# lijx10/SO-Net

Measured on AMD Instinct MI355X. Metric: point-clouds/sec forward, ModelNet40 5k-pt 8x8 SOM, higher is better.
Workload: dtype f32 (operands split into fp16 pieces, 3 fp16 MFMAs per product, f32 accumulate; parity 1e-5)

## Files before the change

so-net_amd/csrc/pointresnet_fused.hip:

```cpp
#include "common.hpp"
#include <stdlib.h>
#include <type_traits>

namespace {


constexpr int PF_THREADS = 256, PF_WAVES = 4;
constexpr int WPTS = 64, TPTS = PF_WAVES * WPTS;
constexpr int T0 = 2, T1 = 4, T2 = 8, T3 = 12;
constexpr int KC2 = 2 * T0, KC3 = 2 * T1, KC4 = 2 * T0 + 2 * T2;
constexpr int MT4 = 3, NPASS = T3 / MT4;
constexpr int GS = 4;
constexpr int NSTG = 24;
constexpr int NTERM = 2;
constexpr int SL1 = 8 , SL2 = KC2 * GS * NTERM, SL3 = (T2 / GS) * KC3 * GS * NTERM;
constexpr int OFF1 = 0, OFF2 = SL1, OFF3 = SL1 + SL2, PRE = SL1 + SL2 + SL3;
constexpr int SL4 = KC4 * MT4 * NTERM;
constexpr int NSLICE = PRE + NPASS * SL4;
constexpr int NSTAGE = NSLICE / NSTG;
static_assert(PRE % NSTG == 0 && SL4 % NSTG == 0 && NSLICE % NSTG == 0, "layer 4 and every pass start on a stage boundary");
static_assert(NSTG % (NTERM * GS) == 0 && NSTG % (NTERM * MT4) == 0 && OFF2 % (NTERM * GS) == 0 && OFF3 % (NTERM * GS) == 0 && T1 == GS && T2 % GS == 0,
              "a step never straddles a stage boundary");
constexpr int NSW = NSTG / PF_WAVES;
static_assert(NSW == 6, "three DMA statements per wave and stage");
// ... 55 lines not shown
        constexpr int g = (I - 8) / 18, k = (I - 8) % 18;
        if constexpr (k < 4) { constexpr int e = 4 * g + k; v.x[e] = pin_fma(v.x[e], s.sc[e].x, s.sc[e].y); }
        else if constexpr (k < 6) { constexpr int e = 4 * g + 2 * (k - 4); if constexpr (RANGE) rm = pin_max3_i32(rm, v.x[e], v.x[e + 1]); }
        else if constexpr (k < 10) { constexpr int e = 4 * g + k - 6; v.x[e] = pin_relu_clamp32(v.x[e]); }
        else if constexpr (k < 12) { constexpr int P = 2 * g + (k - 10); v.h[P] = pin_cvt(v.x[2 * P], v.x[2 * P + 1]); }
        else if constexpr (k < 16) { constexpr int e = 4 * g + (k - 12); v.x[e] = (e & 1) ? pin_res_hi(v.h[e >> 1], v.x[e]) : pin_res_lo(v.h[e >> 1], v.x[e]); }
        else { constexpr int P = 2 * g + (k - 16); v.m[P] = pin_cvt(v.x[2 * P], v.x[2 * P + 1]); }
    } else {
        constexpr int w = I - 44;
        if constexpr (w < 4) agpr_write<R + w>(v.h[w]); else agpr_write<R + w>(v.m[w - 4]);
    }
}
template <int R, bool INPLACE, int I0, int I1, bool RANGE = true> __device__ __forceinline__ void job_ops(JobX &v, const JobSc &s, int &rm) {
    if constexpr (I0 < I1 && I0 < (INPLACE ? JOB_OPS_A : JOB_OPS_V)) { job_op<R, INPLACE, I0, RANGE>(v, s, rm); job_ops<R, INPLACE, I0 + 1, I1, RANGE>(v, s, rm); }
}
__device__ __forceinline__ JobOut job_result(const JobX &v) {
    JobOut o;
    o.h[0] = v.h[0]; o.h[1] = v.h[1]; o.h[2] = v.h[2]; o.h[3] = v.h[3];
    o.m[0] = v.m[0]; o.m[1] = v.m[1]; o.m[2] = v.m[2]; o.m[3] = v.m[3];
    return o;
}

template <int I0, int I1, class F> __device__ __forceinline__ void static_for(F &&f) {
    if constexpr (I0 < I1) { f(std::integral_constant<int, I0>{}); static_for<I0 + 1, I1>(f); }
}
#define SFOR(var, N) static_for<0, (N)>([&](auto var##_c_) __attribute__((always_inline)) { constexpr int var = decltype(var##_c_)::value;
#define SEND });

__global__ __launch_bounds__(256) void pointresnet_pack_kernel(const float *__restrict__ W1, const float *__restrict__ W2,
                                                                const float *__restrict__ W3, const float *__restrict__ W4,
                                                                int Cin0, uint4 *__restrict__ out, unsigned *__restrict__ trailer)
{
    const int t = blockIdx.x * 256 + threadIdx.x;
    if (t >= NSLICE * 64) return;
    RangeAcc wr = {0, 0u};
    const int lane = t & 63, s = t >> 6;
    const int i = lane & 31, h = lane >> 5;
    const float *W = nullptr;
    int Cin = 0, ct = 0, kc = 0, term = 0;
    bool chained = true, valid = true;
    if (s < OFF2) {
        const int u = s - OFF1; term = u % NTERM; kc = 0; ct = u / NTERM; W = W1; Cin = Cin0; chained = false; valid = u < T0 * NTERM;
    } else if (s < OFF3) {
        const int u = s - OFF2; term = u % NTERM; const int mt = (u / NTERM) % GS; kc = (u / (NTERM * GS)) % KC2;
        ct = (u / (NTERM * GS * KC2)) * GS + mt; W = W2; Cin = 32 * T0;
    } else if (s < PRE) {
        const int u = s - OFF3; term = u % NTERM; const int mt = (u / NTERM) % GS; kc = (u / (NTERM * GS)) % KC3;
        ct = (u / (NTERM * GS * KC3)) * GS + mt; W = W3; Cin = 32 * T1;
    } else {
        const int u = (s - PRE) % SL4, pass = (s - PRE) / SL4;
        term = u % NTERM; ct = pass * MT4 + (u / NTERM) % MT4; kc = u / (NTERM * MT4); W = W4; Cin = 32 * (T0 + T2);
    }
    unsigned w[4] = {0, 0, 0, 0};
    if (valid) {
#pragma unroll
        for (int p = 0; p < 4; ++p) {
            float v[2];
#pragma unroll
            for (int z = 0; z < 2; ++z) {
                const int e = 2 * p + z;
                const int c = chained ? kc * 16 + (e & 3) + 8 * (e >> 2) + 4 * h : kc * 16 + 8 * h + e;
                v[z] = c < Cin ? W[(long long)(ct * 32 + i) * Cin + c] : 0.f;
            }
            range_track(wr, 32.f * v[0], 32.f * v[1]);
            const float w0 = v[0] != v[0] ? v[0] : __builtin_fminf(__builtin_fmaxf(32.f * v[0], -F16_MAX32), F16_MAX32);
            const float w1 = v[1] != v[1] ? v[1] : __builtin_fminf(__builtin_fmaxf(32.f * v[1], -F16_MAX32), F16_MAX32);
            unsigned hh, ll;
            p16_split2(w0, w1, hh, ll);
            w[p] = term == 0 ? hh : ll;
        }
    }
    out[(long long)s * 64 + lane] = make_uint4(w[0], w[1], w[2], w[3]);
    range_publish(trailer, wave_umax(range_amax_bits(wr)), lane);
}

constexpr int NSLOT = 3;


struct AF { f16x8 h[GS], l[GS]; };

constexpr int SEG_SLOTS = 16;
constexpr int PCH = 32 * MT4;
constexpr unsigned SEG_INIT = 0x3B85FFFFu;

#ifdef SONET_PROF
constexpr int PROF_N = 32;
__device__ long long g_prof[1024 * PROF_N];
#define PROF_DECL long long prof_[PROF_N] = {}; const long long prof_rt0_ = (long long)__builtin_amdgcn_s_memrealtime(); long long prof_t_ = __builtin_readcyclecounter();
#define PROF_MARK(i) { const long long n_ = __builtin_readcyclecounter(); prof_[i] += n_ - prof_t_; prof_t_ = n_; }
#define PROF_T0 long long pt_ = __builtin_readcyclecounter();
#define PROF_T1(i) { const long long n_ = __builtin_readcyclecounter(); prof_[i] += n_ - pt_; pt_ = n_; }
#define PROF_DUMP prof_[31] = (long long)__builtin_amdgcn_s_memrealtime() - prof_rt0_;  if (lane == 0) { for (int i_ = 0; i_ < PROF_N; ++i_) g_prof[(blockIdx.x * PF_WAVES + wave) * PROF_N + i_] = prof_[i_]; }
#else
#define PROF_DECL
#define PROF_MARK(i)
#define PROF_T0
#define PROF_T1(i)
#define PROF_DUMP
#endif

#define PF_SB __builtin_amdgcn_sched_barrier(0);
#define PF_LDA(base, slice) __builtin_bit_cast(f16x8, (base)[(slice) * 64])
#define AG13(t, c) ((((t) * 2) + (c)) * 16)
#define AG2(t, c) (128 + (((t) * 2) + (c)) * 16)
#define PF_A8(n) "a" #n "0", "a" #n "1", "a" #n "2", "a" #n "3", "a" #n "4", "a" #n "5", "a" #n "6", "a" #n "7", "a" #n "8", "a" #n "9"
#define PF_CLAIM_AGPRS asm volatile("" ::: "a0", "a1", "a2", "a3", "a4", "a5", "a6", "a7", "a8", "a9", PF_A8(1), PF_A8(2), PF_A8(3), PF_A8(4), PF_A8(5), \
        PF_A8(6), PF_A8(7), PF_A8(8), PF_A8(9), PF_A8(10), PF_A8(11), PF_A8(12), PF_A8(13), PF_A8(14), PF_A8(15), PF_A8(16), PF_A8(17), PF_A8(18), PF_A8(19), \
        PF_A8(20), PF_A8(21), PF_A8(22), PF_A8(23), PF_A8(24), "a250", "a251", "a252", "a253", "a254", "a255");

template <bool SEGMAX, bool P16OUT = false>
__global__ __launch_bounds__(PF_THREADS, 1) void pointresnet_fused_kernel(
    const float *__restrict__ x, int Cin0, const uint4 *__restrict__ Wst, const float2 *__restrict__ affine_g ,
    float *__restrict__ y, int L, int tpc , long long ntiles,
    const int32_t *__restrict__ ids_sorted, const int32_t *__restrict__ pos0, unsigned *__restrict__ pooled, float *__restrict__ v0, int M,
    unsigned *__restrict__ partial ,
    unsigned *__restrict__ rlog ,
    void *__restrict__ yp = nullptr )
{
    static_assert(!(SEGMAX && P16OUT), "the pooled variant has no per-point output");
    RangeAcc yr4 = {0, 0u};
    __shared__ uint4 wsm[NSLOT * NSTG][64];
    __shared__ u32x4_t park[PF_WAVES][KC2][2][2][64];
    __shared__ uint4 w1s[T0 * NTERM][64];
    __shared__ __attribute__((aligned(16))) float2 aff[CH_TOTAL];
    __shared__ unsigned bins[SEGMAX ? SEG_SLOTS : 1][SEGMAX ? PCH : 1];

    PF_CLAIM_AGPRS
    const int lane = threadIdx.x & 63;
    const int wave = __builtin_amdgcn_readfirstlane(threadIdx.x >> 6);
    const int j = lane & 31, h = lane >> 5;
    bool l4_unit_lane = true;
    for (int c = threadIdx.x; c < CH_TOTAL; c += PF_THREADS) {
        const float2 v = affine_g[c];
        aff[c] = c < LB4 ? make_float2(v.x * ACC_TO_X32, 32.f * v.y) : make_float2(v.x * ACC_UNSCALE, v.y);
        if (c >= LB4 && v.x != 1.0f) l4_unit_lane = false;
    }
    if constexpr (SEGMAX) {
        for (int i = threadIdx.x; i < SEG_SLOTS * PCH; i += PF_THREADS) (&bins[0][0])[i] = SEG_INIT;
    }
    static_assert(T0 * NTERM * 64 == PF_THREADS, "one 16-byte piece of layer 1's slices per thread");
    w1s[threadIdx.x >> 6][threadIdx.x & 63] = Wst[OFF1 * 64 + threadIdx.x];
    const bool l4_unit = __syncthreads_and(l4_unit_lane) != 0;
    PROF_DECL

    unsigned vow = (unsigned)lane * 16u;
    const unsigned rowB = (unsigned)L * 4u;

    const unsigned wsm_lds = (unsigned)reinterpret_cast<size_t>(&wsm[0][0]);
    const char *dma_g = nullptr;
    unsigned dma_dst = 0;
    auto dma_setup = [&](int n, int slot) __attribute__((always_inline)) {
        const int sn = n % NSTAGE;
        dma_g = reinterpret_cast<const char *>(Wst) + (size_t)(sn * NSTG + wave * NSW) * 1024u;
        dma_dst = wsm_lds + (unsigned)(slot * NSTG + wave * NSW) * 1024u;
    };
    auto dma_pair = [&](auto tc) __attribute__((always_inline)) {
        constexpr int t = decltype(tc)::value;
        const char *g = dma_g + (t / 4) * 4096;
        const unsigned d = dma_dst + (unsigned)(t / 4) * 4096u;
        const unsigned vv = vow;
        if constexpr ((t % 4) == 0) asm volatile("s_mov_b32 m0, %2\n\ts_nop 4\n\tglobal_load_lds_dwordx4 %0, %1\n\tglobal_load_lds_dwordx4 %0, %1 offset:1024" :: "v"(vv), "s"(g), "s"(d) : "memory");
        else                        asm volatile("s_mov_b32 m0, %2\n\ts_nop 4\n\tglobal_load_lds_dwordx4 %0, %1 offset:2048\n\tglobal_load_lds_dwordx4 %0, %1 offset:3072" :: "v"(vv), "s"(g), "s"(d) : "memory");
    };
    auto stage_dma = [&](int n, int slot) __attribute__((always_inline)) {
        dma_setup(n, slot);
        dma_pair(std::integral_constant<int, 0>{}); dma_pair(std::integral_constant<int, 2>{}); dma_pair(std::integral_constant<int, 4>{});
// ... 17 lines not shown
        }
    };
    auto boundary = [&](auto flushc) __attribute__((always_inline)) {
        constexpr bool flush = decltype(flushc)::value;
        PROF_T0
        asm volatile("s_waitcnt vmcnt(0)" ::: "memory");
        PROF_T1(28)
        if constexpr (SEGMAX && flush) asm volatile("s_waitcnt lgkmcnt(0)" ::: "memory");
        __builtin_amdgcn_s_barrier();
        asm volatile("" ::: "memory");
        PROF_T1(29)
        if (!first_boundary) {
            n_cur += 1;
            const int t = slot_cur; slot_cur = slot_nxt; slot_nxt = slot_fill; slot_fill = t;
        }
        first_boundary = false;
        lds_cur = &wsm[slot_cur * NSTG][lane];
        lds_nxt = &wsm[slot_nxt * NSTG][lane];
        if constexpr (SEGMAX && flush) flush_bins();
        dma_setup(n_cur + 2, slot_fill);
    };

    AF af;
#define PF_STEP_HEAD(SIDX, SIDXN, FLUSH)                                                                 \
        constexpr int so_ = (SIDX) % NSTG, son_ = (SIDXN) % NSTG;                                        \
        if constexpr (so_ == 0) boundary(std::integral_constant<bool, (FLUSH)>{});                       \
        const uint4 *nb_ = son_ == 0 ? lds_nxt : lds_cur;
#define PF_STEP_A(NT, SIDX, NTN, SIDXN, AGB, BH0, BM0, BH1, BM1, ZERO, SLOT)                             \
    {                                                                                                    \
        PF_STEP_HEAD(SIDX, SIDXN, false)                                                                 \
        const f16x8 bh_[2] = {as_f16x8(BH0), as_f16x8(BH1)}, bm_[2] = {as_f16x8(BM0), as_f16x8(BM1)};    \
        PF_SB                                                                                            \
        SFOR(q, 2 * (NT)) constexpr int c = q / (NT), u = q % (NT);                                      \
            mfma_agpr<AGB(u, c), (ZERO)>(af.l[u], bh_[c]);                                               \
            if constexpr (so_ == 0 && q < 3) dma_pair(std::integral_constant<int, 2 * q>{});             \
            SLOT(q)                                                                                      \
            PF_SB                                                                                        \
        SEND                                                                                             \
        SFOR(q, 2 * (NT)) constexpr int c = q / (NT), u = q % (NT);                                      \
            mfma_agpr<AGB(u, c), false>(af.h[u], bm_[c]);                                                \
            SLOT(2 * (NT) + q)                                                                           \
            PF_SB                                                                                        \
        SEND                                                                                             \
        SFOR(u, NTN) af.l[u] = PF_LDA(nb_, son_ + NTERM * u + 1); SEND                                   \
        PF_SB                                                                                            \
        SFOR(q, 2 * (NT)) constexpr int c = q / (NT), u = q % (NT);                                      \
            mfma_agpr<AGB(u, c), false>(af.h[u], bh_[c]);                                                \
            SLOT(4 * (NT) + q)                                                                           \
            PF_SB                                                                                        \
        SEND                                                                                             \
        SFOR(u, NTN) af.h[u] = PF_LDA(nb_, son_ + NTERM * u); SEND                                       \
        PF_SB                                                                                            \
    }
#define PF_STEP_V(SIDX, SIDXN, ACC, FROMA, HN0, HN1, BH0, BM0, BH1, BM1, ZERO, FLUSH, SLOT)              \
    {                                                                                                    \
        PF_STEP_HEAD(SIDX, SIDXN, FLUSH)                                                                 \
        const f16x8 bh_[2] = {as_f16x8(BH0), as_f16x8(BH1)}, bm_[2] = {as_f16x8(BM0), as_f16x8(BM1)};    \
        constexpr int hn_[2] = {(HN0), (HN1)};                                                           \
        PF_SB                                                                                            \
        SFOR(q, 2 * MT4) constexpr int c = q / MT4, u = q % MT4;                                         \
            if constexpr (FROMA) mfma_va<hn_[c], SEGMAX>(ACC(u, c), af.l[u]);                            \
            else mfma_vv<(ZERO), SEGMAX>(ACC(u, c), af.l[u], bh_[c]);                                    \
            if constexpr (so_ == 0 && q < 3) dma_pair(std::integral_constant<int, 2 * q>{});             \
            SLOT(q)                                                                                      \
            PF_SB                                                                                        \
        SEND                                                                                             \
        SFOR(q, 2 * MT4) constexpr int c = q / MT4, u = q % MT4;                                         \
            if constexpr (FROMA) mfma_va<hn_[c] + 4, SEGMAX>(ACC(u, c), af.h[u]);                        \
            else mfma_vv<false, SEGMAX>(ACC(u, c), af.h[u], bm_[c]);                                     \
            SLOT(2 * MT4 + q)                                                                            \
            PF_SB                                                                                        \
        SEND                                                                                             \
        SFOR(u, MT4) af.l[u] = PF_LDA(nb_, son_ + NTERM * u + 1); SEND                                   \
        PF_SB                                                                                            \
        SFOR(q, 2 * MT4) constexpr int c = q / MT4, u = q % MT4;                                         \
            if constexpr (FROMA) mfma_va<hn_[c], SEGMAX>(ACC(u, c), af.h[u]);                            \
            else mfma_vv<false, SEGMAX>(ACC(u, c), af.h[u], bh_[c]);                                     \
            SLOT(4 * MT4 + q)                                                                            \
            PF_SB                                                                                        \
        SEND                                                                                             \
        SFOR(u, MT4) af.h[u] = PF_LDA(nb_, son_ + NTERM * u); SEND                                       \
        PF_SB                                                                                            \
    }
#define PF_LOAD_SC(scv, LB, t, Q)                                                                        \
    {                                                                                                    \
        const float4 *ap_ = reinterpret_cast<const float4 *>(&aff[(LB) + 32 * (t) + 16 * (Q) + 4 * h]);  \
        const float4 c0_ = ap_[0], c1_ = ap_[1], c2_ = ap_[4], c3_ = ap_[5];                             \
        scv.sc[0] = make_float2(c0_.x, c0_.y); scv.sc[1] = make_float2(c0_.z, c0_.w);                    \
        scv.sc[2] = make_float2(c1_.x, c1_.y); scv.sc[3] = make_float2(c1_.z, c1_.w);                    \
        scv.sc[4] = make_float2(c2_.x, c2_.y); scv.sc[5] = make_float2(c2_.z, c2_.w);                    \
        scv.sc[6] = make_float2(c3_.x, c3_.y); scv.sc[7] = make_float2(c3_.z, c3_.w);                    \
    }
#ifdef SONET_ABL_NOJOB
#define PF_JOBS_ON false
#else
#define PF_JOBS_ON true
#endif
#define PF_SLOT2(q, OPS, JOPS, INPL, R0, R1)                                                             \
    {                                                                                                    \
        if constexpr (PF_JOBS_ON && (q) >= 2 && (OPS) * ((q) - 2) < 2 * (JOPS)) {                                      \
            constexpr int i0_ = (OPS) * ((q) - 2), i1_ = i0_ + (OPS);                                    \
            if constexpr (i0_ < (JOPS)) job_ops<(R0), (INPL), i0_, (i1_ < (JOPS) ? i1_ : (JOPS))>(jx0_, sc_, rmax_); \
            if constexpr (i1_ > (JOPS)) job_ops<(R1), (INPL), (i0_ > (JOPS) ? i0_ - (JOPS) : 0), i1_ - (JOPS)>(jx1_, sc_, rmax_); \
        }                                                                                                \
    }
#define PF_SLOT1(q, OPS, JOPS, INPL, R0)                                                                 \
    {                                                                                                    \
        if constexpr (PF_JOBS_ON && (q) >= 2 && (OPS) * ((q) - 2) < (JOPS)) {                            \
            constexpr int i0_ = (OPS) * ((q) - 2);                                                       \
            job_ops<(R0), (INPL), i0_, i0_ + (OPS)>(jx0_, sc_, rmax_);                                   \
        }                                                                                                \
    }
    PROF_MARK(0)
    float xin_n[2][8];
    int nid_n[2] = {-1, -1}, n0_n = 0, nlast_n = 0, pos0_n = 0;
    auto prefetch_tile = [&](long long t) __attribute__((always_inline)) {
        t = t < ntiles ? t : ntiles - 1;
        const long long bb = t / tpc;
        const int t0 = (int)(t - bb * tpc) * TPTS;
        const __amdgpu_buffer_rsrc_t rxx = raw_buffer(x + bb * (long long)Cin0 * L, (int)((unsigned)Cin0 * rowB));
#pragma unroll
        for (int c = 0; c < 2; ++c) {
            const int ll0 = t0 + wave * WPTS + 32 * c;
            const bool pvv = ll0 + j < L;
            const int lcc = pvv ? ll0 + j : (ll0 < L ? ll0 : 0);
#pragma unroll
            for (int e = 0; e < 8; ++e)
                xin_n[c][e] = __builtin_bit_cast(float, __builtin_amdgcn_raw_buffer_load_b32(rxx, (unsigned)(8 * h * L + lcc) * 4u, (unsigned)e * rowB, 0));
            if constexpr (SEGMAX) nid_n[c] = pvv ? ids_sorted[bb * (long long)L + ll0 + j] : -1;
        }
        if constexpr (SEGMAX) {
            const int32_t *idb = ids_sorted + bb * (long long)L;
            n0_n = idb[t0];
            nlast_n = idb[(t0 + TPTS - 1 < L ? t0 + TPTS - 1 : L - 1)];
            pos0_n = pos0[bb];
        }
    };
    prefetch_tile(blockIdx.x);
    int rmax_ = 0;
    unsigned xin_r = 0u;
    u32x4_t *const park_w = &park[wave][0][0][0][lane];
#define PF_PARK(kc, c, piece) park_w[(((kc) * 2 + (c)) * 2 + (piece)) * 64]

    SFOR(u, T0) af.l[u] = PF_LDA(lds_cur, NTERM * u + 1); af.h[u] = PF_LDA(lds_cur, NTERM * u); SEND

    for (long long tile = blockIdx.x; tile < ntiles; tile += gridDim.x) {
        const long long b = tile / tpc;
        const int t0w = (int)(tile - b * tpc) * TPTS + wave * WPTS;
        bool pv[2]; int lc[2];
#pragma unroll
        for (int c = 0; c < 2; ++c) {
            const int l0 = t0w + 32 * c;
            pv[c] = l0 + j < L;
            lc[c] = pv[c] ? l0 + j : (l0 < L ? l0 : 0);
        }
        int nid[2] = {-1, -1}, n0 = 0, nslots = 0, jpos0[2] = {-1, -1};
        if constexpr (SEGMAX) {
            nid[0] = nid_n[0]; nid[1] = nid_n[1];
            n0 = n0_n;
            nslots = nlast_n - n0_n + 1 < SEG_SLOTS ? nlast_n - n0_n + 1 : SEG_SLOTS;
#pragma unroll
            for (int c = 0; c < 2; ++c) {
                const int p0 = pos0_n - (t0w + 32 * c);
                jpos0[c] = (p0 >= 0 && p0 < 32) ? p0 : -1;
            }
        }
        u32x4_t xh[2], xm[2];
#pragma unroll
        for (int c = 0; c < 2; ++c) {
#pragma unroll
            for (int p = 0; p < 4; ++p) {
                unsigned a0, a1;
                asm volatile("v_and_b32 %0, 0x7fffffff, %1" : "=v"(a0) : "v"(xin_n[c][2 * p]));
                asm volatile("v_and_b32 %0, 0x7fffffff, %1" : "=v"(a1) : "v"(xin_n[c][2 * p + 1]));
                asm volatile("v_max3_u32 %0, %0, %1, %2" : "+v"(xin_r) : "v"(a0), "v"(a1));
            }
            split_input(xin_n[c], xh[c], xm[c]);
        }
        PROF_MARK(1)
#define NOSLOT(q)
        PF_STEP_A(T0, OFF1, GS, OFF2, AG13, xh[0], xm[0], xh[1], xm[1], true, NOSLOT)
        JobOut a1[T0][2][2];
        {
            asm volatile("s_nop 15" ::: );
            JobSc sc_; JobX jx0_, jx1_;
            PF_LOAD_SC(sc_, LB1, 0, 0)
            job_ops<AG13(0, 0), false, 0, JOB_OPS_V>(jx0_, sc_, rmax_);
            job_ops<AG13(0, 1), false, 0, JOB_OPS_V>(jx1_, sc_, rmax_);
            a1[0][0][0] = job_result(jx0_); a1[0][0][1] = job_result(jx1_);
        }
        PROF_MARK(6)
        SFOR(k, KC2)
            constexpr int tk = k >> 1, qk = k & 1;
            constexpr int kn = k + 1, tn = (kn >> 1) & 1, qn = kn & 1;
            constexpr int sidx = OFF2 + k * NTERM * GS;
            JobSc sc_; JobX jx0_, jx1_;
            if constexpr (k + 1 < KC2) PF_LOAD_SC(sc_, LB1, tn, qn)
#define SLOT_L2(q) { if constexpr (k + 1 < KC2) { PF_SLOT2(q, 4, JOB_OPS_V, false, AG13(tn, 0) + 8 * qn, AG13(tn, 1) + 8 * qn) \
                       if constexpr ((q) == 23) { a1[tn][qn][0] = job_result(jx0_); a1[tn][qn][1] = job_result(jx1_); } } }
            PF_STEP_A(GS, sidx, GS, sidx + NTERM * GS, AG2, a1[tk][qk][0].h, a1[tk][qk][0].m, a1[tk][qk][1].h, a1[tk][qk][1].m, (k == 0), SLOT_L2)
#undef SLOT_L2
        SEND
        JobOut a2[T1][2][2];
        {
            asm volatile("s_nop 15" ::: );
            JobSc sc_; JobX jx0_, jx1_;
            PF_LOAD_SC(sc_, LB2, 0, 0)
            job_ops<AG2(0, 0), false, 0, JOB_OPS_V>(jx0_, sc_, rmax_);
            job_ops<AG2(0, 1), false, 0, JOB_OPS_V>(jx1_, sc_, rmax_);
            a2[0][0][0] = job_result(jx0_); a2[0][0][1] = job_result(jx1_);
        }
        PROF_MARK(7)
#define AG3A(u, c) AG13(u, c)
#define AG3B(u, c) AG13(GS + (u), c)
        u32x4_t pbh[2], pbm[2];
        SFOR(k, KC3)
            constexpr int tk = k >> 1, qk = k & 1;
            if constexpr (k + 1 == KC3) {
                pbh[0] = PF_PARK(0, 0, 0); pbm[0] = PF_PARK(0, 0, 1);
                pbh[1] = PF_PARK(0, 1, 0); pbm[1] = PF_PARK(0, 1, 1);
            }
            constexpr int kn = k + 1, tn = (kn >> 1) & 3, qn = kn & 1;
            constexpr int sidx = OFF3 + k * NTERM * GS;
            JobSc sc_; JobX jx0_, jx1_;
            if constexpr (k + 1 < KC3) PF_LOAD_SC(sc_, LB2, tn, qn)
#define SLOT_L3A(q) { if constexpr (k + 1 < KC3) { PF_SLOT2(q, 4, JOB_OPS_V, false, AG2(tn, 0) + 8 * qn, AG2(tn, 1) + 8 * qn) \
                        if constexpr ((q) == 23) { a2[tn][qn][0] = job_result(jx0_); a2[tn][qn][1] = job_result(jx1_); } } }
            PF_STEP_A(GS, sidx, GS, sidx + NTERM * GS, AG3A, a2[tk][qk][0].h, a2[tk][qk][0].m, a2[tk][qk][1].h, a2[tk][qk][1].m, (k == 0), SLOT_L3A)
#undef SLOT_L3A
            if constexpr (k < KC2) {
                PF_PARK(k, 0, 0) = a2[tk][qk][0].h; PF_PARK(k, 0, 1) = a2[tk][qk][0].m;
                PF_PARK(k, 1, 0) = a2[tk][qk][1].h; PF_PARK(k, 1, 1) = a2[tk][qk][1].m;
            }
        SEND
        PROF_MARK(8)
        float xagain[2][8];
        SFOR(k, KC3)
            constexpr int tk = k >> 1, qk = k & 1;
            constexpr int sidx = OFF3 + (KC3 + k) * NTERM * GS;
            constexpr int ntn = k + 1 < KC3 ? GS : MT4;
            constexpr bool cur_park = k < KC2, nxt_park = k + 1 < KC2;
            JobSc sc_; JobX jx0_, jx1_;
            PF_LOAD_SC(sc_, LB3, tk, qk)
            const u32x4_t ch0 = cur_park ? pbh[0] : a2[tk][qk][0].h, cm0 = cur_park ? pbm[0] : a2[tk][qk][0].m;
            const u32x4_t ch1 = cur_park ? pbh[1] : a2[tk][qk][1].h, cm1 = cur_park ? pbm[1] : a2[tk][qk][1].m;
            if constexpr (nxt_park) {
                pbh[0] = PF_PARK(k + 1, 0, 0); pbm[0] = PF_PARK(k + 1, 0, 1);
                pbh[1] = PF_PARK(k + 1, 1, 0); pbm[1] = PF_PARK(k + 1, 1, 1);
            }
            if constexpr (k + 1 == KC3) {
                const __amdgpu_buffer_rsrc_t rxx = raw_buffer(x + b * (long long)Cin0 * L, (int)((unsigned)Cin0 * rowB));
#pragma unroll
                for (int c = 0; c < 2; ++c)
#pragma unroll
                    for (int e = 0; e < 8; ++e)
                        xagain[c][e] = __builtin_bit_cast(float, __builtin_amdgcn_raw_buffer_load_b32(rxx, (unsigned)(8 * h * L + lc[c]) * 4u, (unsigned)e * rowB, 0));
            }
#define SLOT_L3B(q) { PF_SLOT2(q, 5, JOB_OPS_A, true, AG13(tk, 0) + 8 * qk, AG13(tk, 1) + 8 * qk) }
            PF_STEP_A(GS, sidx, ntn, sidx + NTERM * GS, AG3B, ch0, cm0, ch1, cm1, (k == 0), SLOT_L3B)
#undef SLOT_L3B
        SEND
        PROF_MARK(9)
        {
            f32x16 r1[T0][2];
            f16x8 wh[T0], wl[T0];
            SFOR(u, T0) wl[u] = __builtin_bit_cast(f16x8, w1s[NTERM * u + 1][lane]); wh[u] = __builtin_bit_cast(f16x8, w1s[NTERM * u][lane]); SEND
            u32x4_t xh0, xm0, xh1, xm1;
            split_input(xagain[0], xh0, xm0);
            split_input(xagain[1], xh1, xm1);
            const f16x8 bh_[2] = {as_f16x8(xh0), as_f16x8(xh1)}, bm_[2] = {as_f16x8(xm0), as_f16x8(xm1)};
            PF_SB
            SFOR(q, 2 * T0) constexpr int c = q / T0, u = q % T0; mfma_vv<true, false>(r1[u][c], wl[u], bh_[c]); PF_SB SEND
            SFOR(q, 2 * T0) constexpr int c = q / T0, u = q % T0; mfma_vv<false, false>(r1[u][c], wh[u], bm_[c]); PF_SB SEND
            SFOR(q, 2 * T0) constexpr int c = q / T0, u = q % T0; mfma_vv<false, false>(r1[u][c], wh[u], bh_[c]); PF_SB SEND
            asm volatile("s_nop 15" ::: );
            int rdummy = 0;
            SFOR(kk, KC2)
                constexpr int tk = kk >> 1, qk = kk & 1;
                JobSc sc_;
                PF_LOAD_SC(sc_, LB1, tk, qk)
                SFOR(c, 2)
                    JobX jx_;
                    SFOR(i, 8) jx_.x[i] = r1[tk][c][8 * qk + i]; SEND
                    job_ops<0, false, 8, JOB_OPS_V, false>(jx_, sc_, rdummy);
                    const JobOut o = job_result(jx_);
                    PF_PARK(kk, c, 0) = o.h; PF_PARK(kk, c, 1) = o.m;
                    if constexpr (kk == 0) { pbh[c] = o.h; pbm[c] = o.m; }
                SEND
            SEND
        }
        PROF_MARK(2)
        const __amdgpu_buffer_rsrc_t ry = raw_buffer(y ? y + b * (long long)(32 * T3) * L : x, y ? (int)((unsigned)(32 * T3) * rowB) : 0);
        const __amdgpu_buffer_rsrc_t ryp = raw_buffer(P16OUT ? static_cast<char *>(yp) + b * (long long)(2 * T3) * 64 * L : nullptr, P16OUT ? (int)((unsigned)(2 * T3) * 64u * (unsigned)L) : 0);
#define ACC4(u, c) acc[u][c]
#define PF_L4_BODY(JOBS)                                                                                 \
            SFOR(kc, KC4)                                                                                \
                constexpr int sidx = PRE + kc * NTERM * MT4;                                             \
                constexpr int kn = (kc + 1) % KC4;                                                       \
                constexpr bool cur_park = kc < KC2, nxt_park = kn < KC2;                                 \
                constexpr int t3 = cur_park ? 0 : (kc - KC2) >> 1, q3 = cur_park ? 0 : (kc - KC2) & 1;   \
                constexpr int jt = T2 / 2 + kc / 4, jq = (kc >> 1) & 1, jc = kc & 1;                     \
                constexpr bool job = (JOBS) && kc < 16;                                                  \
                JobSc sc_; JobX jx0_;                                                                    \
                if constexpr (job) PF_LOAD_SC(sc_, LB3, (job ? jt : 0), jq)                              \
                const u32x4_t ch0 = pbh[0], cm0 = pbm[0], ch1 = pbh[1], cm1 = pbm[1];                    \
                if constexpr (nxt_park) {                         \
                    pbh[0] = PF_PARK(kn, 0, 0); pbm[0] = PF_PARK(kn, 0, 1);                              \
                    pbh[1] = PF_PARK(kn, 1, 0); pbm[1] = PF_PARK(kn, 1, 1);                              \
                }                                                                                        \
                PF_STEP_V(sidx, sidx + NTERM * MT4, ACC4, !cur_park, AG13(t3, 0) + 8 * q3, AG13(t3, 1) + 8 * q3, ch0, cm0, ch1, cm1, (kc == 0), (kc == 0), SLOT_L4) \
            SEND
#define SLOT_L4(q) { if constexpr (job) { PF_SLOT1(q, 4, JOB_OPS_A, true, AG13((job ? jt : 0), jc) + 8 * jq) } }
        auto epilogue = [&](f32x16 (&acc)[MT4][2], const int pass) __attribute__((always_inline)) {
#ifdef SONET_ABL_NOEPI
            if (M != 12345) return;
#endif
            asm volatile("s_nop 15" ::: );
            if constexpr (SEGMAX) {
                float bias4[MT4];
#pragma unroll
                for (int mt = 0; mt < MT4; ++mt) {
                    const float2 ss = aff[LB4 + (pass * MT4 + mt) * 32 + j];
                    bias4[mt] = ss.y;
                    if (!l4_unit) {
#pragma unroll
                        for (int c = 0; c < 2; ++c)
#pragma unroll
                            for (int r = 0; r < 16; ++r) acc[mt][c][r] = __fmaf_rn(acc[mt][c][r], ss.x, ss.y);
                    }
                }
#pragma unroll
                for (int c = 0; c < 2; ++c) {
                    if (jpos0[c] >= 0) {
#pragma unroll
                        for (int r = 0; r < 16; ++r)
                            if ((r & 3) + 8 * (r >> 2) + 4 * h == jpos0[c]) {
#pragma unroll
                                for (int mt = 0; mt < MT4; ++mt) v0[b * (32 * T3) + (pass * MT4 + mt) * 32 + j] = l4_unit ? __fmaf_rn(acc[mt][c][r], ACC_UNSCALE, bias4[mt]) : acc[mt][c][r];
                            }
                    }
                    auto publish = [&](int node, float (&mx)[MT4]) __attribute__((always_inline)) {
                        if (l4_unit) {
#pragma unroll
                            for (int mt = 0; mt < MT4; ++mt) mx[mt] = __fmaf_rn(mx[mt], ACC_UNSCALE, bias4[mt]);
                        }
                        const int slot = node - n0;
                        if (slot < SEG_SLOTS) {
#pragma unroll
                            for (int mt = 0; mt < MT4; ++mt) atomicMax(&bins[slot][32 * mt + j], ord_f32(__float_as_uint(mx[mt])));
                        } else {
                            unsigned *gdst = pooled + ((long long)b * M + node) * (32 * T3) + pass * PCH;
#pragma unroll
                            for (int mt = 0; mt < MT4; ++mt) atomicMax(gdst + 32 * mt + j, ord_f32(__float_as_uint(mx[mt])));
                        }
                    };
                    unsigned remaining = (unsigned)__ballot(pv[c]);
                    if (remaining == 0xFFFFFFFFu) {
                        const int node_a = __builtin_amdgcn_readlane(nid[c], 0), node_b = __builtin_amdgcn_readlane(nid[c], 31);
                        const int e = __builtin_popcount((unsigned)__ballot(nid[c] == node_a));
                        if (node_a != node_b && __builtin_amdgcn_readlane(nid[c], e & 31) == node_b) {
                            float ma[MT4], mb[MT4];
#pragma unroll
                            for (int mt = 0; mt < MT4; ++mt) ma[mt] = mb[mt] = -__builtin_inff();
#pragma unroll
                            for (int r = 0; r < 16; r += 2) {
                                const int prow = (r & 3) + 8 * (r >> 2) + 4 * h;
                                const bool in0 = prow < e, in1 = prow + 1 < e;
#pragma unroll
                                for (int mt = 0; mt < MT4; ++mt) {
                                    const float a0 = in0 ? acc[mt][c][r] : -__builtin_inff(), a1 = in1 ? acc[mt][c][r + 1] : -__builtin_inff();
                                    const float b0 = in0 ? -__builtin_inff() : acc[mt][c][r], b1 = in1 ? -__builtin_inff() : acc[mt][c][r + 1];
                                    asm("v_max3_f32 %0, %1, %2, %3" : "=v"(ma[mt]) : "v"(ma[mt]), "v"(a0), "v"(a1));
                                    asm("v_max3_f32 %0, %1, %2, %3" : "=v"(mb[mt]) : "v"(mb[mt]), "v"(b0), "v"(b1));
                                }
                            }
                            publish(node_a, ma);
                            publish(node_b, mb);
                            remaining = 0u;
                        }
                    }
                    while (remaining != 0u) {
                        const int s0 = __builtin_ctz(remaining);
                        const int node = __builtin_amdgcn_readlane(nid[c], s0);
                        const unsigned segmask = (unsigned)__ballot(pv[c] && nid[c] == node);
                        remaining &= ~segmask;
                        const int e0 = s0 + __builtin_popcount(segmask);
                        const bool whole = (s0 == 0 && e0 == 32);
                        float mx[MT4];
                        if (whole) {
#pragma unroll
                            for (int mt = 0; mt < MT4; ++mt) {
                                float m;
                                asm("v_max_f32 %0, %1, %2" : "=v"(m) : "v"(acc[mt][c][0]), "v"(acc[mt][c][1]));
#pragma unroll
                                for (int r = 2; r < 16; r += 2) asm("v_max3_f32 %0, %1, %2, %3" : "=v"(m) : "v"(m), "v"(acc[mt][c][r]), "v"(acc[mt][c][r + 1]));
                                mx[mt] = m;
                            }
                        } else {
#pragma unroll
                            for (int mt = 0; mt < MT4; ++mt) mx[mt] = -__builtin_inff();
                            const unsigned nrows = (unsigned)(e0 - s0);
#pragma unroll
                            for (int r = 0; r < 16; r += 2) {
                                const int prow = (r & 3) + 8 * (r >> 2) + 4 * h;
                                const bool in0 = (unsigned)(prow - s0) < nrows, in1 = (unsigned)(prow + 1 - s0) < nrows;
#pragma unroll
                                for (int mt = 0; mt < MT4; ++mt) {
                                    const float v0_ = in0 ? acc[mt][c][r] : -__builtin_inff(), v1_ = in1 ? acc[mt][c][r + 1] : -__builtin_inff();
                                    asm("v_max3_f32 %0, %1, %2, %3" : "=v"(mx[mt]) : "v"(mx[mt]), "v"(v0_), "v"(v1_));
                                }
                            }
                        }
                        publish(node, mx);
                    }
                }
                pend_n = nslots * PCH;
                pend = partial + ((tile * NPASS + pass) * SEG_SLOTS) * (long long)PCH;
            } else {
#pragma unroll
                for (int c = 0; c < 2; ++c) {
                    if (!pv[c]) continue;
#pragma unroll
                    for (int mt = 0; mt < MT4; ++mt) {
                        const int ct = pass * MT4 + mt;
                        const unsigned so_tile = (unsigned)(ct * 32) * rowB;
                        float vv[16];
#pragma unroll
                        for (int r = 0; r < 16; ++r) {
                            const int orow = (r & 3) + 8 * (r >> 2);
                            const float2 ss = aff[LB4 + ct * 32 + orow + 4 * h];
                            const float v = __fmaf_rn(acc[mt][c][r], ss.x, ss.y);
                            vv[r] = v;
                            __builtin_amdgcn_raw_buffer_store_b32(__builtin_bit_cast(int, v), ry, (unsigned)(4 * h * L + lc[c]) * 4u,
                                                                  so_tile + (unsigned)orow * rowB, 0);
                        }
                        if constexpr (P16OUT) {
#pragma unroll
                            for (int q = 0; q < 2; ++q) {
                                unsigned hh[4], mm[4];
#pragma unroll
                                for (int p = 0; p < 4; ++p) {
                                    const float x0 = vv[8 * q + 2 * p], x1 = vv[8 * q + 2 * p + 1];
                                    range_track(yr4, x0, x1);
                                    p16_split_pair(x0, x1, hh[p], mm[p]);
                                }
                                const unsigned so = (unsigned)((ct * 2 + q) * 2) * (unsigned)L * 32u;
                                const u32x4_t hv = {hh[0], hh[1], hh[2], hh[3]}, mv = {mm[0], mm[1], mm[2], mm[3]};
                                __builtin_amdgcn_raw_buffer_store_b128(hv, ryp, (unsigned)(h * L + lc[c]) * 16u, so, 0);
                                __builtin_amdgcn_raw_buffer_store_b128(mv, ryp, (unsigned)(h * L + lc[c]) * 16u, so + (unsigned)L * 32u, 0);
                            }
                        }
                    }
                }
            }
        };
        {
            f32x16 acc[MT4][2];
            PF_L4_BODY(true)
            prefetch_tile(tile + gridDim.x);
            PROF_MARK(10)
            epilogue(acc, 0);
            PROF_MARK(4)
        }
        for (int pass = 1; pass < NPASS; ++pass) {
            f32x16 acc[MT4][2];
            PF_L4_BODY(false)
            PROF_MARK(3)
            epilogue(acc, pass);
            PROF_MARK(4)
        }
#undef SLOT_L4
    }
    asm volatile("s_waitcnt vmcnt(0)" ::: "memory");
    if constexpr (SEGMAX) {
        __syncthreads();
        flush_bins();
    }
    if (rlog != nullptr) {
        range_publish(rlog, wave_umax(xin_r), lane);
        unsigned rb = wave_umax((unsigned)(rmax_ > 0 ? rmax_ : 0));
        rb = rb > (5u << 23) ? rb - (5u << 23) : 0u;
        if constexpr (P16OUT) {
            const unsigned ob = wave_umax(range_amax_bits(yr4));
            rb = rb > ob ? rb : ob;
        }
        range_publish(rlog + 2, rb, lane);
        if (blockIdx.x == 0 && threadIdx.x == 0) atomicMax(rlog + 1, reinterpret_cast<const unsigned *>(Wst + (long long)NSLICE * 64)[0]);
    }
    PROF_MARK(5)
    PROF_DUMP
}

__global__ __launch_bounds__(256) void pooled_init_kernel(unsigned *__restrict__ pooled, long long n) {
    const long long t = (long long)blockIdx.x * 256 + threadIdx.x;
    if (t < n) pooled[t] = SEG_INIT;
}

__global__ __launch_bounds__(256) void pooled_decode_kernel(const unsigned *__restrict__ pooled, const unsigned *__restrict__ partial,
                                                             const int32_t *__restrict__ ids_sorted, const int32_t *__restrict__ node_off,
                                                             const int32_t *__restrict__ count, const float *__restrict__ v0,
                                                             float *__restrict__ out, int M, int L, int tpc,
                                                             uint4 *__restrict__ out_p16, unsigned *__restrict__ rlog)
{
    constexpr int C = 32 * T3;
    __shared__ float tile[32][33];
    const long long b = blockIdx.z;
    const int m0 = blockIdx.y * 32, c0 = blockIdx.x * 32;
    const int lx = threadIdx.x & 31, ly = threadIdx.x >> 5;
    const int c = c0 + lx;
    const int pass = c / PCH, cl = c - pass * PCH;
#pragma unroll
    for (int i = 0; i < 4; ++i) {
        const int m = m0 + ly + 8 * i;
        if (m < M) {
            unsigned key = pooled[(b * M + m) * C + c];
            const int cnt = count[b * M + m];
            if (cnt > 0) {
                const int off = node_off[b * M + m];
                for (int tl = off / TPTS; tl <= (off + cnt - 1) / TPTS; ++tl) {
                    const int slot = m - ids_sorted[b * L + tl * TPTS];
                    if (slot < SEG_SLOTS) {
                        const unsigned k2 = partial[((((b * tpc + tl) * NPASS + pass) * SEG_SLOTS) + slot) * (long long)PCH + cl];
                        key = k2 > key ? k2 : key;
                    }
                }
            }
            float v;
            if (key > SEG_INIT) v = __uint_as_float((key & 0x80000000u) ? (key ^ 0x80000000u) : ~key);
            else v = v0[b * C + c];
            tile[ly + 8 * i][lx] = v;
        }
    }
    __syncthreads();
#pragma unroll
    for (int i = 0; i < 4; ++i) {
        const int cc = c0 + ly + 8 * i, m = m0 + lx;
        if (m < M) out[(b * C + cc) * M + m] = tile[lx][ly + 8 * i];
    }
    if (out_p16 != nullptr && threadIdx.x < 128) {
        const int node = threadIdx.x & 31, qq = (threadIdx.x >> 6) & 1, hh = (threadIdx.x >> 5) & 1;
        const int m = m0 + node;
        RangeAcc xr = {0, 0u};
        if (m < M) {
            const long long BM = ((long long)gridDim.z * M + 127) / 128 * 128, l = b * M + m;
            float v[8];
#pragma unroll
            for (int e = 0; e < 8; ++e) v[e] = tile[node][16 * qq + 4 * hh + (e & 3) + 8 * (e >> 2)];
            unsigned hv[4], mv[4];
#pragma unroll
            for (int q = 0; q < 4; ++q) {
                range_track(xr, v[2 * q], v[2 * q + 1]);
                p16_split_pair(v[2 * q], v[2 * q + 1], hv[q], mv[q]);
            }
            const int kc = c0 / 16 + qq;
// ... 2 lines not shown
        }
        if (rlog != nullptr) range_publish(rlog + 2, wave_umax(range_amax_bits(xr)), (int)(threadIdx.x & 63));
    }
}

long long persistent_grid(long long ntiles, int cus) {
    static const int free_cus = [] { int v = 0; sonet::knob_int("SONET_FUSED_FREE_CUS", &v); return v; }();
    if (ntiles <= cus) return ntiles;
    if (free_cus == 0) return cus;
    const long long rounds = (ntiles + cus - 1) / cus;
    long long grid = (ntiles + rounds - 1) / rounds;
    if (free_cus > 0 && grid > cus - free_cus) grid = cus - free_cus > 1 ? cus - free_cus : 1;
    return free_cus > 0 || free_cus == -1 ? grid : cus;
}

}

extern "C" size_t sonet_pointresnet_pack_size(void) { return (size_t)NSLICE * 1024 + 64; }

extern "C" int sonet_pointresnet_pack(const float *W1, const float *W2, const float *W3, const float *W4, int Cin0,
                                      void *stream_out, sonet_stream_t stream)
{
    const char *what = "sonet_pointresnet_pack";
    SONET_REQUIRE(W1 && W2 && W3 && W4 && stream_out, "%s: NULL pointer", what);
    SONET_REQUIRE(Cin0 >= 1 && Cin0 <= 16, "%s: Cin0=%d must be in [1, 16]", what, Cin0);
    unsigned *trailer = reinterpret_cast<unsigned *>(reinterpret_cast<char *>(stream_out) + (size_t)NSLICE * 1024);
    if (hipMemsetAsync(trailer, 0, 64, sonet::as_stream(stream)) != hipSuccess) return sonet::fail(SONET_ERR_LAUNCH, "%s: memset failed", what);
    hipLaunchKernelGGL(pointresnet_pack_kernel, dim3(sonet::ceil_div(NSLICE * 64, 256)), dim3(256), 0, sonet::as_stream(stream),
                       W1, W2, W3, W4, Cin0, reinterpret_cast<uint4 *>(stream_out), trailer);
    return sonet::launched(what);
}

extern "C" int sonet_pointresnet_fused_f32(const float *x, int Cin0, const void *wstream, const float *affine,
                                           float *y, int B, int L, sonet_stream_t stream)
{
    const char *what = "sonet_pointresnet_fused_f32";
    SONET_REQUIRE(x && wstream && affine && y, "%s: NULL pointer", what);
    SONET_REQUIRE(B > 0 && L > 0 && Cin0 >= 1 && Cin0 <= 16, "%s: bad size B=%d L=%d Cin0=%d", what, B, L, Cin0);
    if ((double)(32 * T3) * L * 4.0 >= 4.0e9) return sonet::fail(SONET_ERR_UNSUPPORTED, "%s: a per-cloud panel exceeds 4 GiB", what);
    const int tpc = sonet::ceil_div(L, TPTS);
    const long long ntiles = (long long)B * tpc;
    const long long grid = persistent_grid(ntiles, sonet::cu_count(1));
    hipLaunchKernelGGL((pointresnet_fused_kernel<false>), dim3((unsigned)grid), dim3(PF_THREADS), 0, sonet::as_stream(stream),
                       x, Cin0, reinterpret_cast<const uint4 *>(wstream), reinterpret_cast<const float2 *>(affine), y, L, tpc, ntiles,
                       (const int32_t *)nullptr, (const int32_t *)nullptr, (unsigned *)nullptr, (float *)nullptr, 0, (unsigned *)nullptr, sonet::range_log());
    return sonet::launched(what);
}

extern "C" int sonet_pointresnet_fused_p16_f32(const float *x, int Cin0, const void *wstream, const float *affine,
                                               float *y, void *yp, int B, int L, sonet_stream_t stream)
{
    const char *what = "sonet_pointresnet_fused_p16_f32";
    SONET_REQUIRE(x && wstream && affine && yp, "%s: NULL pointer", what);
    SONET_REQUIRE(B > 0 && L > 0 && Cin0 >= 1 && Cin0 <= 16, "%s: bad size B=%d L=%d Cin0=%d", what, B, L, Cin0);
    if ((double)(32 * T3) * L * 4.0 >= 2.0e9) return sonet::fail(SONET_ERR_UNSUPPORTED, "%s: a per-cloud panel exceeds 2 GiB", what);
    const int tpc = sonet::ceil_div(L, TPTS);
    const long long ntiles = (long long)B * tpc;
    const long long grid = persistent_grid(ntiles, sonet::cu_count(1));
    hipLaunchKernelGGL((pointresnet_fused_kernel<false, true>), dim3((unsigned)grid), dim3(PF_THREADS), 0, sonet::as_stream(stream),
                       x, Cin0, reinterpret_cast<const uint4 *>(wstream), reinterpret_cast<const float2 *>(affine), y, L, tpc, ntiles,
                       (const int32_t *)nullptr, (const int32_t *)nullptr, (unsigned *)nullptr, (float *)nullptr, 0, (unsigned *)nullptr, sonet::range_log(), yp);
    return sonet::launched(what);
}

extern "C" size_t sonet_pointresnet_pool_ws_size(int B, int L, int M)
{
    if (B <= 0 || L <= 0 || M <= 0) return 0;
    const long long ntiles = (long long)B * sonet::ceil_div(L, TPTS);
    return (size_t)((long long)B * M * (32 * T3) + ntiles * NPASS * SEG_SLOTS * PCH) * 4 + (size_t)B * (32 * T3) * 4;
}

static int fused_pool_impl(const char *what, const float *x_sorted, int Cin0, const void *wstream, const float *affine,
                           const int32_t *ids_sorted, const int32_t *pos0, const int32_t *node_off,
                           const int32_t *count, void *ws, float *out, void *out_p16, int B, int L, int M, sonet_stream_t stream)
{
    SONET_REQUIRE(x_sorted && wstream && affine && ids_sorted && pos0 && node_off && count && ws && out, "%s: NULL pointer", what);
    SONET_REQUIRE(B > 0 && L > 0 && M > 0 && Cin0 >= 1 && Cin0 <= 16, "%s: bad size B=%d L=%d M=%d Cin0=%d", what, B, L, M, Cin0);
    if (B > 65535) return sonet::fail(SONET_ERR_UNSUPPORTED, "%s: B=%d > 65535", what, B);
    if (16.0 * L * 4.0 >= 4.0e9) return sonet::fail(SONET_ERR_UNSUPPORTED, "%s: a per-cloud input panel of 16 rows exceeds 4 GiB", what);
    hipStream_t st = sonet::as_stream(stream);
    const long long npool = (long long)B * M * (32 * T3);
    const int tpc = sonet::ceil_div(L, TPTS);
    const long long ntiles = (long long)B * tpc;
    unsigned *pooled_ws = reinterpret_cast<unsigned *>(ws);
    unsigned *partial_ws = pooled_ws + npool;
    float *v0_ws = reinterpret_cast<float *>(partial_ws + ntiles * NPASS * SEG_SLOTS * PCH);
    hipLaunchKernelGGL(pooled_init_kernel, dim3((unsigned)sonet::ceil_div64(npool, 256)), dim3(256), 0, st, pooled_ws, npool);
    const long long grid = persistent_grid(ntiles, sonet::cu_count(1));
    hipLaunchKernelGGL((pointresnet_fused_kernel<true>), dim3((unsigned)grid), dim3(PF_THREADS), 0, st,
                       x_sorted, Cin0, reinterpret_cast<const uint4 *>(wstream), reinterpret_cast<const float2 *>(affine), (float *)nullptr,
                       L, tpc, ntiles, ids_sorted, pos0, pooled_ws, v0_ws, M, partial_ws, sonet::range_log());
    hipLaunchKernelGGL(pooled_decode_kernel, dim3((unsigned)(32 * T3 / 32), (unsigned)sonet::ceil_div(M, 32), (unsigned)B), dim3(256), 0, st,
                       pooled_ws, partial_ws, ids_sorted, node_off, count, v0_ws, out, M, L, tpc, reinterpret_cast<uint4 *>(out_p16), sonet::range_log());
    return sonet::launched(what);
}

extern "C" int sonet_pointresnet_fused_pool_f32(const float *x_sorted, int Cin0, const void *wstream, const float *affine,
                                                const int32_t *ids_sorted, const int32_t *pos0, const int32_t *node_off,
                                                const int32_t *count, void *ws, float *out, int B, int L, int M, sonet_stream_t stream)
{
    return fused_pool_impl("sonet_pointresnet_fused_pool_f32", x_sorted, Cin0, wstream, affine, ids_sorted, pos0, node_off, count, ws, out, nullptr, B, L, M, stream);
}

extern "C" int sonet_pointresnet_fused_pool_p16_f32(const float *x_sorted, int Cin0, const void *wstream, const float *affine,
                                                    const int32_t *ids_sorted, const int32_t *pos0, const int32_t *node_off,
                                                    const int32_t *count, void *ws, float *out, void *out_p16, int B, int L, int M, sonet_stream_t stream)
{
    const char *what = "sonet_pointresnet_fused_pool_p16_f32";
    SONET_REQUIRE(out_p16, "%s: NULL pointer", what);
    return fused_pool_impl(what, x_sorted, Cin0, wstream, affine, ids_sorted, pos0, node_off, count, ws, out, out_p16, B, L, M, stream);
}

#ifdef SONET_PROF
extern "C" int sonet_prof_read(long long *host, int n)
{
    return hipMemcpyFromSymbol(host, HIP_SYMBOL(g_prof), sizeof(long long) * (size_t)n, 0, hipMemcpyDeviceToHost) == hipSuccess ? 0 : 1;
}
#endif
```

Before: 78030.

## Overlap segment max-pool reduction with next pass MFMAs and track tile coordinates incrementally

Adds an optional path, on only when SONET_VARIANTS is defined, that interleaves the per-pass segment max-pool reduction (max3, scale and bias, ordered-int encode, LDS atomicMax) for wave-uniform tiles into the MFMA slots of the last and first layer-4 steps, in place of running a separate epilogue. Separately, the segmax kernel now keeps batch and tile indices incrementally instead of 64-bit divisions per tile, and the host rejects tile counts of 2^31 or more. The overlap path adds register pressure and inline asm. Without the define, only the incremental indexing takes effect.

Result: no change. 77930 (-0.1%).

```diff
diff --git a/so-net_amd/csrc/pointresnet_fused.hip b/so-net_amd/csrc/pointresnet_fused.hip
--- a/so-net_amd/csrc/pointresnet_fused.hip
+++ b/so-net_amd/csrc/pointresnet_fused.hip
@@ -161,6 +161,11 @@
 constexpr int SEG_SLOTS = 16;
 constexpr int PCH = 32 * MT4;
 constexpr unsigned SEG_INIT = 0x3B85FFFFu;
+#ifdef SONET_VARIANTS
+constexpr bool PF_POOL_OVERLAP = true;
+#else
+constexpr bool PF_POOL_OVERLAP = false;
+#endif
 
 #ifdef SONET_PROF
 constexpr int PROF_N = 32;
@@ -344,6 +349,30 @@
         SFOR(u, MT4) af.h[u] = PF_LDA(nb_, son_ + NTERM * u); SEND                                       \
         PF_SB                                                                                            \
     }
+#define PF_STEP_VC(SIDX, SIDXN, ACC, FROMA, HN0, HN1, BH0, BM0, BH1, BM1, ZERO, SLOT)                    \
+    {                                                                                                    \
+        PF_STEP_HEAD(SIDX, SIDXN, false)                                                                 \
+        const f16x8 bh_[2] = {as_f16x8(BH0), as_f16x8(BH1)}, bm_[2] = {as_f16x8(BM0), as_f16x8(BM1)};    \
+        constexpr int hn_[2] = {(HN0), (HN1)};                                                           \
+        PF_SB                                                                                            \
+        SFOR(q, 2 * MT4) constexpr int c = q / MT4, u = q % MT4;                                         \
+            if constexpr (FROMA) mfma_va<hn_[c], SEGMAX>(ACC(u, c), af.l[u]);                            \
+            else mfma_vv<(ZERO), SEGMAX>(ACC(u, c), af.l[u], bh_[c]);                                    \
+            if constexpr (so_ == 0 && q < 3) dma_pair(std::integral_constant<int, 2 * q>{});             \
+            SLOT(3 * q)                                                                                  \
+            PF_SB                                                                                        \
+            if constexpr (FROMA) mfma_va<hn_[c] + 4, SEGMAX>(ACC(u, c), af.h[u]);                        \
+            else mfma_vv<false, SEGMAX>(ACC(u, c), af.h[u], bm_[c]);                                     \
+            SLOT(3 * q + 1)                                                                              \
+            PF_SB                                                                                        \
+            if constexpr (c == 1) { af.l[u] = PF_LDA(nb_, son_ + NTERM * u + 1); PF_SB }                 \
+            if constexpr (FROMA) mfma_va<hn_[c], SEGMAX>(ACC(u, c), af.h[u]);                            \
+            else mfma_vv<false, SEGMAX>(ACC(u, c), af.h[u], bh_[c]);                                     \
+            SLOT(3 * q + 2)                                                                              \
+            PF_SB                                                                                        \
+            if constexpr (c == 1) { af.h[u] = PF_LDA(nb_, son_ + NTERM * u); PF_SB }                     \
+        SEND                                                                                             \
+    }
 #define PF_LOAD_SC(scv, LB, t, Q)                                                                        \
     {                                                                                                    \
         const float4 *ap_ = reinterpret_cast<const float4 *>(&aff[(LB) + 32 * (t) + 16 * (Q) + 4 * h]);  \
@@ -376,10 +405,24 @@
     PROF_MARK(0)
     float xin_n[2][8];
     int nid_n[2] = {-1, -1}, n0_n = 0, nlast_n = 0, pos0_n = 0;
+    int g_q = 0, g_r = 0, b_last = 0, b_n = 0, tl_n = 0;
+    if constexpr (SEGMAX) {
+        g_q = (int)(gridDim.x / (unsigned)tpc); g_r = (int)(gridDim.x % (unsigned)tpc);
+        b_last = (int)((unsigned)(ntiles - 1) / (unsigned)tpc);
+        b_n = (int)(blockIdx.x / (unsigned)tpc); tl_n = (int)(blockIdx.x % (unsigned)tpc);
+    }
     auto prefetch_tile = [&](long long t) __attribute__((always_inline)) {
-        t = t < ntiles ? t : ntiles - 1;
-        const long long bb = t / tpc;
-        const int t0 = (int)(t - bb * tpc) * TPTS;
+        long long bb;
+        int t0;
+        if constexpr (SEGMAX) {
+            if (t >= ntiles) { b_n = b_last; tl_n = tpc - 1; }
+            bb = b_n;
+            t0 = tl_n * TPTS;
+        } else {
+            t = t < ntiles ? t : ntiles - 1;
+            bb = t / tpc;
+            t0 = (int)(t - bb * tpc) * TPTS;
+        }
         const __amdgpu_buffer_rsrc_t rxx = raw_buffer(x + bb * (long long)Cin0 * L, (int)((unsigned)Cin0 * rowB));
 #pragma unroll
         for (int c = 0; c < 2; ++c) {
@@ -407,8 +450,8 @@
     SFOR(u, T0) af.l[u] = PF_LDA(lds_cur, NTERM * u + 1); af.h[u] = PF_LDA(lds_cur, NTERM * u); SEND
 
     for (long long tile = blockIdx.x; tile < ntiles; tile += gridDim.x) {
-        const long long b = tile / tpc;
-        const int t0w = (int)(tile - b * tpc) * TPTS + wave * WPTS;
+        const long long b = SEGMAX ? (long long)b_n : tile / tpc;
+        const int t0w = (SEGMAX ? tl_n : (int)(tile - b * tpc)) * TPTS + wave * WPTS;
         bool pv[2]; int lc[2];
 #pragma unroll
         for (int c = 0; c < 2; ++c) {
@@ -426,6 +469,17 @@
                 const int p0 = pos0_n - (t0w + 32 * c);
                 jpos0[c] = (p0 >= 0 && p0 < 32) ? p0 : -1;
             }
+        }
+        bool fastw = false;
+        int fslot[2] = {0, 0};
+        unsigned fmask = 0u;
+        if constexpr (SEGMAX && PF_POOL_OVERLAP) {
+            const int na0 = __builtin_amdgcn_readfirstlane(nid[0]), na1 = __builtin_amdgcn_readfirstlane(nid[1]);
+            const bool w0 = __ballot(pv[0] && nid[0] == na0) == ~0ull, w1 = __ballot(pv[1] && nid[1] == na1) == ~0ull;
+            const int n0u = __builtin_amdgcn_readfirstlane(n0);
+            fastw = __builtin_amdgcn_readfirstlane((int)(l4_unit && w0 && w1 && jpos0[0] < 0 && jpos0[1] < 0 && na1 - n0u < SEG_SLOTS)) != 0;
+            fslot[0] = fastw ? na0 - n0u : 0; fslot[1] = fastw ? na1 - n0u : 0;
+            fmask = fastw ? 0xFFFFFFFFu : 0u;
         }
         u32x4_t xh[2], xm[2];
 #pragma unroll
@@ -555,7 +609,7 @@
         const __amdgpu_buffer_rsrc_t ry = raw_buffer(y ? y + b * (long long)(32 * T3) * L : x, y ? (int)((unsigned)(32 * T3) * rowB) : 0);
         const __amdgpu_buffer_rsrc_t ryp = raw_buffer(P16OUT ? static_cast<char *>(yp) + b * (long long)(2 * T3) * 64 * L : nullptr, P16OUT ? (int)((unsigned)(2 * T3) * 64u * (unsigned)L) : 0);
 #define ACC4(u, c) acc[u][c]
-#define PF_L4_BODY(JOBS)                                                                                 \
+#define PF_L4_BODY(JOBS, OVL)                                                                            \
             SFOR(kc, KC4)                                                                                \
                 constexpr int sidx = PRE + kc * NTERM * MT4;                                             \
                 constexpr int kn = (kc + 1) % KC4;                                                       \
@@ -570,7 +624,17 @@
                     pbh[0] = PF_PARK(kn, 0, 0); pbm[0] = PF_PARK(kn, 0, 1);                              \
                     pbh[1] = PF_PARK(kn, 1, 0); pbm[1] = PF_PARK(kn, 1, 1);                              \
                 }                                                                                        \
-                PF_STEP_V(sidx, sidx + NTERM * MT4, ACC4, !cur_park, AG13(t3, 0) + 8 * q3, AG13(t3, 1) + 8 * q3, ch0, cm0, ch1, cm1, (kc == 0), (kc == 0), SLOT_L4) \
+                 \
+                constexpr bool flush_ = SEGMAX && PF_POOL_OVERLAP ? kc == NSTG / (NTERM * MT4) : kc == 0; \
+                constexpr bool drain_ = (OVL) && kc == KC4 - 1, fill_ = (OVL) && !(JOBS) && kc == 0;     \
+                if constexpr (drain_) {                                                                  \
+                    POOL_DRAIN_HEAD                                                                      \
+                    PF_STEP_VC(sidx, sidx + NTERM * MT4, ACC4, true, AG13(t3, 0) + 8 * q3, AG13(t3, 1) + 8 * q3, ch0, cm0, ch1, cm1, false, SLOT_DRAIN) \
+                } else if constexpr (fill_) {                                                            \
+                    PF_STEP_VC(sidx, sidx + NTERM * MT4, ACC4, false, 0, 0, ch0, cm0, ch1, cm1, true, SLOT_FILL) \
+                } else {                                                                                 \
+                    PF_STEP_V(sidx, sidx + NTERM * MT4, ACC4, !cur_park, AG13(t3, 0) + 8 * q3, AG13(t3, 1) + 8 * q3, ch0, cm0, ch1, cm1, (kc == 0), flush_, SLOT_L4) \
+                }                                                                                        \
             SEND
 #define SLOT_L4(q) { if constexpr (job) { PF_SLOT1(q, 4, JOB_OPS_A, true, AG13((job ? jt : 0), jc) + 8 * jq) } }
         auto epilogue = [&](f32x16 (&acc)[MT4][2], const int pass) __attribute__((always_inline)) {
@@ -716,9 +780,60 @@
                 }
             }
         };
+        f32x16 acc[MT4][2];
+        struct { float m, bias; unsigned t; } ps_ = {0.f, 0.f, 0u};
+        int pool_pass_ = 0;
+        constexpr int POOL_OPS = 16, POOL_N = 2 * MT4 * POOL_OPS, POOL_RATE = 4, POOL_S0 = 4, POOL_DRAINED = POOL_RATE * (6 * MT4 - POOL_S0);
+        auto pool_op = [&](auto ic) __attribute__((always_inline)) {
+            constexpr int I = decltype(ic)::value, k = I / POOL_OPS, o = I % POOL_OPS, c = k / MT4, u = k % MT4;
+            if constexpr (o == 0) {
+                ps_.bias = aff[LB4 + (pool_pass_ * MT4 + u) * 32 + j].y;
+                asm volatile("v_max_f32 %0, %1, %2" : "=v"(ps_.m) : "v"(acc[u][c][0]), "v"(acc[u][c][1]));
+            }
+            else if constexpr (o < 8) asm volatile("v_max3_f32 %0, %1, %2, %3" : "=v"(ps_.m) : "v"(ps_.m), "v"(acc[u][c][2 * o]), "v"(acc[u][c][2 * o + 1]));
+            else if constexpr (o == 8) asm volatile("v_fma_f32 %0, %1, %2, %3" : "=v"(ps_.m) : "v"(ps_.m), "s"(ACC_UNSCALE), "v"(ps_.bias));
+            else if constexpr (o == 9) asm volatile("v_cmp_eq_u32 vcc, 0x80000000, %0\n\tv_cndmask_b32_e64 %0, %0, 0, vcc" : "+v"(ps_.m) :: "vcc");
+            else if constexpr (o == 10) asm volatile("v_ashrrev_i32 %0, 31, %1" : "=v"(ps_.t) : "v"(ps_.m));
+            else if constexpr (o == 11) asm volatile("v_or_b32 %0, 0x80000000, %0" : "+v"(ps_.t));
+            else if constexpr (o == 12) asm volatile("v_xor_b32 %0, %1, %0" : "+v"(ps_.t) : "v"(ps_.m));
+            else if constexpr (o == 13) asm volatile("v_and_b32 %0, 0x7fffffff, %0" : "+v"(ps_.m));
+            else if constexpr (o == 14) asm volatile("v_cmp_lt_u32 vcc, 0x7f800000, %1\n\tv_cndmask_b32_e64 %0, %0, 0, vcc\n\tv_and_b32 %0, %2, %0" : "+v"(ps_.t) : "v"(ps_.m), "s"(fmask) : "vcc");
+            else atomicMax(&bins[c == 0 ? fslot[0] : fslot[1]][32 * u + j], ps_.t);
+        };
+#define POOL_DRAIN_HEAD                                                                                  \
+        pool_pass_ = pass_;                                                                          \
+        pend_n = nslots * PCH;                                                                       \
+        pend = partial + ((tile * NPASS + pass_) * SEG_SLOTS) * (long long)PCH;
+#define SLOT_DRAIN(i) { if constexpr ((i) >= POOL_S0) static_for<POOL_RATE * ((i) - POOL_S0), POOL_RATE * ((i) + 1 - POOL_S0)>(pool_op); }
+#define SLOT_FILL(i) { if constexpr (POOL_DRAINED + POOL_RATE * (i) < POOL_N) static_for<POOL_DRAINED + POOL_RATE * (i), POOL_DRAINED + POOL_RATE * ((i) + 1)>(pool_op); }
+        static_assert(POOL_N % POOL_RATE == 0 && POOL_DRAINED < POOL_N && POOL_N - POOL_DRAINED <= POOL_RATE * 6 * MT4, "the stream ends inside the fill step");
+        static_assert(POOL_RATE * (3 * 3 + 2 + 2 - POOL_S0) <= POOL_OPS * 3 && POOL_OPS >= POOL_RATE * 3, "a statement never runs before its accumulator is complete");
+        int pass_ = 0;
+        if constexpr (SEGMAX && PF_POOL_OVERLAP) {
+            PF_L4_BODY(true, true)
+            tl_n += g_r; b_n += g_q;
+            if (tl_n >= tpc) { tl_n -= tpc; b_n += 1; }
+            prefetch_tile(tile + gridDim.x);
+            PROF_MARK(10)
+            if (!fastw) epilogue(acc, 0);
+            PROF_MARK(4)
+            for (pass_ = 1; pass_ < NPASS; ++pass_) {
+                PF_L4_BODY(false, true)
+                PROF_MARK(3)
+                if (!fastw) epilogue(acc, pass_);
+                PROF_MARK(4)
+            }
+            asm volatile("s_nop 15" ::: );
+            static_for<POOL_DRAINED, POOL_N>(pool_op);
+            PROF_MARK(4)
+        } else {
         {
             f32x16 acc[MT4][2];
-            PF_L4_BODY(true)
+            PF_L4_BODY(true, false)
+            if constexpr (SEGMAX) {
+                tl_n += g_r; b_n += g_q;
+                if (tl_n >= tpc) { tl_n -= tpc; b_n += 1; }
+            }
             prefetch_tile(tile + gridDim.x);
             PROF_MARK(10)
             epilogue(acc, 0);
@@ -726,12 +841,16 @@
         }
         for (int pass = 1; pass < NPASS; ++pass) {
             f32x16 acc[MT4][2];
-            PF_L4_BODY(false)
+            PF_L4_BODY(false, false)
             PROF_MARK(3)
             epilogue(acc, pass);
             PROF_MARK(4)
         }
+        }
 #undef SLOT_L4
+#undef SLOT_FILL
+#undef SLOT_DRAIN
+#undef POOL_DRAIN_HEAD
     }
     asm volatile("s_waitcnt vmcnt(0)" ::: "memory");
     if constexpr (SEGMAX) {
@@ -900,6 +1019,7 @@
     const long long npool = (long long)B * M * (32 * T3);
     const int tpc = sonet::ceil_div(L, TPTS);
     const long long ntiles = (long long)B * tpc;
+    if (ntiles >= (1LL << 31)) return sonet::fail(SONET_ERR_UNSUPPORTED, "%s: B=%d x %d tiles per cloud is 2^31 tiles or more", what, B, tpc);
     unsigned *pooled_ws = reinterpret_cast<unsigned *>(ws);
     unsigned *partial_ws = pooled_ws + npool;
     float *v0_ws = reinterpret_cast<float *>(partial_ws + ntiles * NPASS * SEG_SLOTS * PCH);
```
